# amoretti86/PSVO

Measured on AMD Instinct MI355X. Metric: particle-steps/sec, higher is better.
Workload: dtype f32

## Files before the change

psvo_amd/csrc/bsim_bwd2_impl.h:

```cpp
#pragma once
#define PSVO_BSIM_BWD_V2_UNIT 1
#include "bsim_bwd_impl.h"

namespace psvo {
PSVO_TIMERS_DEFINE(bsim_bwd2)

template <class T>
using gptr = T __attribute__((address_space(1)))*;
template <class T>
__device__ __forceinline__ gptr<T> as_global(T* p) { return (gptr<T>)p; }
template <class T>
__device__ __forceinline__ gptr<T> as_global(unsigned long long p) { return (gptr<T>)p; }
__device__ __forceinline__ float ldf(gptr<const float> base, unsigned off) {
    return *reinterpret_cast<gptr<const float>>(reinterpret_cast<gptr<const char>>(base) + off);
}
__device__ __forceinline__ int ldi(gptr<const int32_t> base, unsigned off) {
    return *reinterpret_cast<gptr<const int32_t>>(reinterpret_cast<gptr<const char>>(base) + off);
}
__device__ __forceinline__ void stf(gptr<float> base, unsigned off, float v) {
    *reinterpret_cast<gptr<float>>(reinterpret_cast<gptr<char>>(base) + off) = v;
}
#define PSVO_GARG(args_type, field) ::psvo::as_global(PSVO_ARG(args_type, field))

__device__ __forceinline__ float swap_add32(float lo, float hi) {
    asm volatile("s_nop 1\n\tv_permlane32_swap_b32 %0, %1" : "+v"(lo), "+v"(hi));
    return lo + hi;
}
__device__ __forceinline__ float swap_add16(float lo, float hi) {
    asm volatile("s_nop 1\n\tv_permlane16_swap_b32 %0, %1" : "+v"(lo), "+v"(hi));
    return lo + hi;
}
__device__ __forceinline__ float row_sum16(float v) {
    v += dpp_mov<0x128, 0xF, 0xF, true>(v, v);
    v += dpp_mov<0x124, 0xF, 0xF, true>(v, v);
    v += dpp_mov<0x122, 0xF, 0xF, true>(v, v);
    v += dpp_mov<0x121, 0xF, 0xF, true>(v, v);
    return v;
}

__device__ __forceinline__ float rs_bit3(float lo, float hi) {
    float r;
    asm volatile("s_nop 1\n\t"
                 "v_add_f32_dpp %0, %1, %1 row_ror:8 row_mask:0xf bank_mask:0x3\n\t"
                 "v_add_f32_dpp %0, %2, %2 row_ror:8 row_mask:0xf bank_mask:0xc"
                 : "=&v"(r) : "v"(lo), "v"(hi));
    return r;
}
__device__ __forceinline__ float rs_bit2(float lo, float hi) {
    float r;
    asm volatile("s_nop 1\n\t"
                 "v_add_f32_dpp %0, %1, %1 row_shl:4 row_mask:0xf bank_mask:0x5\n\t"
                 "v_add_f32_dpp %0, %2, %2 row_shr:4 row_mask:0xf bank_mask:0xa"
                 : "=&v"(r) : "v"(lo), "v"(hi));
    return r;
}
template <int K>
__device__ __forceinline__ void row_reduce_scatter(const float (&v)[4 * K], float (&out)[K]) {
    float h[2 * K];
#pragma unroll
    for (int i = 0; i < 2 * K; ++i) h[i] = rs_bit3(v[i], v[2 * K + i]);
#pragma unroll
    for (int i = 0; i < K; ++i) out[i] = group_sum<4>(rs_bit2(h[i], h[K + i]));
}

typedef float f4v __attribute__((ext_vector_type(4)));
typedef __bf16 bf8v __attribute__((ext_vector_type(8)));

__device__ __forceinline__ void bf16_split3(float v, unsigned& h, unsigned& m, unsigned& l) {
    const unsigned hb = __float_as_uint(v) & 0xffff0000u;
    const float r = v - __uint_as_float(hb);
    const unsigned mb = __float_as_uint(r) & 0xffff0000u;
    const float r2 = r - __uint_as_float(mb);
    h = hb >> 16;
    m = mb >> 16;
    l = __float_as_uint(r2) >> 16;
}
__device__ __forceinline__ uint4 bf16x3_a(float v) {
    unsigned h, m, l;
    bf16_split3(v, h, m, l);
    return make_uint4(h | (h << 16), m | (h << 16), l | (m << 16), m | (l << 16));
}
__device__ __forceinline__ uint4 bf16x3_b(float v) {
    unsigned h, m, l;
    bf16_split3(v, h, m, l);
    return make_uint4(h | (m << 16), h | (l << 16), h | (m << 16), l | (m << 16));
}

template <int DX, int DY, int H, int M, int JM>
__global__ void __launch_bounds__(256, 2) bsim_bwd2_kernel(const BsimBwdArgs a) {
    using MQ = MlpLds<DX, H, DX, 1>;
    using MG = MlpLds<DX, H, DY, 1>;
    using AC = BAcc<DX, DY>;
    constexpr int PS = (JM == 3) ? 20 : (DX == 4 && JM == 0) ? 5 : BTileSlot<DX>::kFloats;
    constexpr int FO = (JM == 3) ? 16 : 0;
    constexpr int NA = DX + 1;
    constexpr int PART = 2;
    constexpr int G = M * PART;
    constexpr int CPW = 64 / G;
    constexpr int CM = CPW * M;
    constexpr int NF = DX + 2;
    constexpr int UVS = (2 * DX + 3) & ~3;
    constexpr int JC = (JM == 0 && DX == 4) ? 2 : (JM || DX >= 3) ? 4 : 8;
    constexpr bool RO = (DX == 4) && (JM == 0);
    constexpr bool kSplitTile = (DX == 4) && (JM == 0);
    static_assert(CM == 32 && (M % 4) == 0, "two lanes per (chain, m): M in {4, 8, 16, 32}");
    extern __shared__ __attribute__((aligned(16))) float smem[];

    const int tid = threadIdx.x, lane = tid & 63, wave = tid >> 6;
    constexpr int NTB = 256, nwv = 4;
    const int B = a.B, T = a.T, N = a.N;
    const int NP = ((N + 127) / 128) * 128;
    const int nch = NP / (16 * JC);
    const int b = blockIdx.y, blk = blockIdx.x, nblk = gridDim.x;
    constexpr int cpb = nwv * CPW;
    const int cl = lane / G, part = (lane / M) & 1, m = lane % M;
    const bool h0 = (part == 0);
    const int n_raw = blk * cpb + wave * CPW + cl;
    const bool valid = n_raw < N;
    const int n = valid ? n_raw : N - 1;
    const bool srow = valid && h0;
    const bool lead = srow && (m == 0);
    const int j16 = lane & 15, g = lane >> 4;

    float* wf = smem;
    float* wg = wf + MQ::kSize;
    float* wqi = wg + MG::kSize;
    float* tile = wqi + MQ::kSize;
    float* jacc = tile + 2 * NP * PS;
    float* xch = jacc + nwv * NA * NP;
    float* uvx = xch + nwv * NF * CM;
    float* red = uvx + nwv * CM * UVS;
    float* const xw = xch + wave * NF * CM;
    float* const uw = uvx + wave * CM * UVS;
    float* const ja = jacc + wave * NA * NP;

    MQ::load(wf, a.f, tid, NTB);
    MG::load(wg, a.g, tid, NTB);
    MQ::load(wqi, a.q1inv, tid, NTB);

    const float kappa = sqrtf(0.5f * kLog2e);
    float isf[DX], rp[DX], isfk[DX], isg[DY];
#pragma unroll
    for (int d = 0; d < DX; ++d) {
        isf[d] = 1.f / a.sig_f[d];
        rp[d] = isf[d] * kappa;
        isfk[d] = isf[d] / kappa;
    }
    float ikap2 = 1.f / (kappa * kappa);
#pragma unroll
    for (int e = 0; e < DY; ++e) isg[e] = 1.f / a.sig_g[e];
    float pc[DX], pic[DX], pi1[DX], pi2[DX];
#pragma unroll
    for (int d = 0; d < DX; ++d) {
        pi1[d] = 1.f / a.sig_q1inv[d];
        pi2[d] = 1.f / a.sig_bq2[d];
        pic[d] = pi1[d] + pi2[d];
        pc[d] = 1.f / pic[d];
    }
    float s_init[DX], is_init[DX], i_isig[DX], im[DX], mi[DX];
#pragma unroll
    for (int d = 0; d < DX; ++d) {
        s_init[d] = a.sig_init[d];
        is_init[d] = 1.f / s_init[d];
        i_isig[d] = 1.f / a.isig[d];
        im[d] = a.imean[b * DX + d];
        mi[d] = a.minit[b * DX + d];
    }
    if constexpr (DX <= 2) {
        keep_in_vgpr(isf); keep_in_vgpr(rp); keep_in_vgpr(isfk); keep_in_vgpr(isg); keep_in_vgpr(ikap2);
        keep_in_vgpr(pc); keep_in_vgpr(pic); keep_in_vgpr(pi1); keep_in_vgpr(pi2);
    }
    const float ninf = -__builtin_huge_valf();
    const float aw = valid ? as_global(a.dscore)[(size_t)b * N + n] : 0.f;

// ... 769 lines not shown
```

psvo_amd/csrc/bsim_fwd.hip:

```cpp
#include "common.h"

namespace psvo {
inline namespace PSVO_LNS {
PSVO_TIMERS_DEFINE(bsim_fwd)


struct BsimArgs {
    int B, T, N;
    int emission;
    psvo_mlp f, g, q1inv;
    const float *X, *Fm, *logW, *lse;
    const float *sig_f, *sig_g, *sig_q1inv, *sig_bq2;
    const float *bmu2, *minit, *sig_init, *imean, *isig;
    const float *obs, *eps_b, *u_b;
    const int32_t* sel_in;
    float *bwX, *flp, *glp, *Omega;
    int32_t* sel_out;
    float* score;
    float *lam2_all, *om_all, *mu1_all;
};

template <int DX>
struct TileSlot {
    static constexpr int kFloats = (DX <= 3) ? 4 : 8;
};

__device__ __forceinline__ float quad_bcast(float v, int lane, int i) { return __shfl(v, (lane & ~3) | i); }

__device__ __forceinline__ void lse2_merge(float& m, float& s, float m2, float s2) {
    const float nm = fmaxf(m, m2);
    const float a = (m == nm) ? 1.f : exp2_fast(m - nm);
    const float b = (m2 == nm) ? 1.f : exp2_fast(m2 - nm);
    s = s * a + s2 * b;
    m = nm;
}

template <int DX, int DY, int H, int M, int HS>
__global__ void __launch_bounds__(256) bsim_fwd_kernel(const BsimArgs a) {
    using MQ = MlpLds<DX, H, DX, PSVO_L>;
    using MG = MlpLds<DX, H, DY, PSVO_L>;
    constexpr int PS = TileSlot<DX>::kFloats;
    constexpr int kMaxStage = 4;
    constexpr bool kRolled = (2 * MQ::kSize + MG::kSize) > 330;
    constexpr bool kPeel = (DX <= 3);
    extern __shared__ __attribute__((aligned(16))) float smem[];

    const int tid = threadIdx.x, lane = tid & 63;
    const int NTB = blockDim.x;
    const int B = a.B, T = a.T, N = a.N;
    const int NP = ((N + 16 * HS - 1) / (16 * HS)) * (16 * HS);
    const int b = blockIdx.y;
    constexpr int G = M * HS;
    const int cpb = NTB / G;
    const int cl = tid / G, hpart = (tid % G) / M, m = tid % M, q = m & 3;
    const bool lead = (m == 0) && (hpart == 0);
    const int n_raw = blockIdx.x * cpb + cl;
    const bool valid = n_raw < N;
    const int n = valid ? n_raw : N - 1;
    const int gbase = lane - m;

    float* wf = smem;
    float* wg = wf + MQ::kSize;
    float* wqi = wg + MG::kSize;
    float* tile = wqi + MQ::kSize;

    MQ::load(wf, a.f, tid, NTB);
    MG::load(wg, a.g, tid, NTB);
    MQ::load(wqi, a.q1inv, tid, NTB);

    float isf[DX], rp[DX], isg[DY];
    float kf = -DX * kHalfLog2Pi, kg = -DY * kHalfLog2Pi;
    const float rscale = sqrtf(0.5f * kLog2e);
#pragma unroll
    for (int d = 0; d < DX; ++d) {
        const float s = a.sig_f[d];
        isf[d] = 1.f / s;
        rp[d] = isf[d] * rscale;
        kf -= logf(s);
    }
#pragma unroll
    for (int e = 0; e < DY; ++e) {
        const float s = a.sig_g[e];
        isg[e] = 1.f / s;
        kg -= logf(s);
    }
    float pc[DX], pic[DX], pi1[DX], pi2[DX];
    float kq = -DX * kHalfLog2Pi;
#pragma unroll
    for (int d = 0; d < DX; ++d) {
        pi1[d] = 1.f / a.sig_q1inv[d];
        pi2[d] = 1.f / a.sig_bq2[d];
        pic[d] = pi1[d] + pi2[d];
        pc[d] = 1.f / pic[d];
        kq -= logf(pc[d]);
    }
    float s_init[DX], is_init[DX], i_isig[DX], im[DX], mi[DX];
    float kinit = -DX * kHalfLog2Pi, kiota = -DX * kHalfLog2Pi;
#pragma unroll
    for (int d = 0; d < DX; ++d) {
        s_init[d] = a.sig_init[d];
        is_init[d] = 1.f / s_init[d];
        kinit -= logf(s_init[d]);
        i_isig[d] = 1.f / a.isig[d];
        kiota -= logf(a.isig[d]);
        im[d] = a.imean[b * DX + d];
        mi[d] = a.minit[b * DX + d];
    }
    const float logM = logf((float)M);
    const float ninf = -__builtin_huge_valf();

    float st[kMaxStage][DX + 1], st_l = 0.f;
    auto stage_load = [&](int tt) {
        const size_t tb = (size_t)tt * B + b;
        st_l = a.lse[tb];
#pragma unroll
        for (int r = 0; r < kMaxStage; ++r) {
            const int j = tid + r * NTB;
            if (j < NP) {
                const int jc = j < N ? j : N - 1;
#pragma unroll
                for (int d = 0; d < DX; ++d) st[r][d] = a.Fm[(tb * DX + d) * N + jc];
                st[r][DX] = a.logW[tb * N + jc];
            }
        }
    };
    auto stage_store = [&](float* buf) {
#pragma unroll
        for (int r = 0; r < kMaxStage; ++r) {
            const int j = tid + r * NTB;
            if (j < NP) {
                float F[DX];
#pragma unroll
                for (int d = 0; d < DX; ++d) F[d] = st[r][d] * rp[d];
                const float W = j < N ? (st[r][DX] - st_l) * kLog2e : ninf;
                if constexpr (DX <= 3) {
                    float4 v;
                    v.x = F[0];
                    v.y = DX > 1 ? F[DX > 1 ? 1 : 0] : 0.f;
                    v.z = DX > 2 ? F[DX > 2 ? 2 : 0] : 0.f;
                    v.w = W;
                    *reinterpret_cast<float4*>(buf + j * PS) = v;
                } else {
                    *reinterpret_cast<float4*>(buf + j * PS) = make_float4(F[0], F[1], F[2], F[3]);
                    *reinterpret_cast<float4*>(buf + j * PS + 4) = make_float4(W, 0.f, 0.f, 0.f);
                }
            }
        }
    };

    if (T >= 2) {
        stage_load(T - 2);
        stage_store(tile);
    }

    float eps_c[DX], bmu_c[DX], obs_c[DY], u_c = 0.f;
    int sel_c = 0;
    auto load_inputs = [&](int t, float (&e)[DX], float (&bm)[DX], float (&o)[DY], float& uu, int& ss) {
        const size_t tb = (size_t)t * B + b;
#pragma unroll
        for (int d = 0; d < DX; ++d) {
            e[d] = a.eps_b[((tb * DX + d) * N + n) * M + m];
            bm[d] = a.bmu2[tb * DX + d];
        }
#pragma unroll
        for (int k = 0; k < DY; ++k) o[k] = a.obs[tb * DY + k];
        if (a.sel_in) ss = a.sel_in[tb * N + n];
        else uu = a.u_b[tb * N + n];
    };
    load_inputs(T - 1, eps_c, bmu_c, obs_c, u_c, sel_c);
    __syncthreads();

    float xp[DX];
#pragma unroll
    for (int d = 0; d < DX; ++d) xp[d] = 0.f;
    float score = 0.f;

    SEC_INIT(bsim_fwd)
    auto step = [&](auto last_tag, auto zero_tag, const int t) {
        SEC(0);
        const size_t tb = (size_t)t * B + b;
        const float* cur = tile + ((T - 1 - t) & 1) * NP * PS;
        float* nxt = tile + ((T - t) & 1) * NP * PS;
        const bool last = last_tag;
        const bool tzero = zero_tag;

        float eps_n[DX], bmu_n[DX], obs_n[DY], u_n = 0.f;
        int sel_n = 0;
        if (!tzero) load_inputs(t - 1, eps_n, bmu_n, obs_n, u_n, sel_n);
        if (t >= 2) stage_load(t - 2);

        SEC(1);
        float x[DX], q_lp;
        if (last) {
            float mu[DX];
#pragma unroll
            for (int d = 0; d < DX; ++d) {
                mu[d] = mi[d];
                x[d] = fmaf(s_init[d], eps_c[d], mu[d]);
            }
            q_lp = diag_lp<DX>(x, mu, is_init, kinit);
            if (a.mu1_all && valid && lead) {
#pragma unroll
                for (int d = 0; d < DX; ++d) a.mu1_all[(tb * DX + d) * N + n] = 0.f;
            }
        } else {
            float m1[DX], mu[DX];
            {
                constexpr int kQS = (H / 4 < G) ? H / 4 : G;
                MQ::template eval_part<kQS>(wqi, (tid % G) & (kQS - 1), xp, m1);
#pragma unroll
                for (int d = 0; d < DX; ++d) m1[d] = group_sum<kQS>(m1[d]);
            }
            if (a.mu1_all && valid && lead) {
#pragma unroll
                for (int d = 0; d < DX; ++d) a.mu1_all[(tb * DX + d) * N + n] = m1[d];
            }
#pragma unroll
            for (int d = 0; d < DX; ++d) {
                mu[d] = pc[d] * fmaf(pi1[d], m1[d], pi2[d] * bmu_c[d]);
                x[d] = fmaf(pc[d], eps_c[d], mu[d]);
            }
            q_lp = diag_lp<DX>(x, mu, pic, kq);
        }

        SEC(2);
        float phi = 0.f;
        if (!last) {
            float fmx[DX];
            if constexpr (HS == 1) {
                MQ::template eval<kRolled>(wf, x, fmx);
            } else {
                MQ::template eval_part<HS, ilog2(M)>(wf, hpart, x, fmx);
#pragma unroll
                for (int d = 0; d < DX; ++d) fmx[d] += xor_lane<M>(fmx[d]);
            }
            phi = diag_lp<DX>(xp, fmx, isf, kf);
        }
        float gm[DY];
        if constexpr (HS == 1) {
            MG::template eval<kRolled>(wg, x, gm);
        } else {
            MG::template eval_part<HS, ilog2(M)>(wg, hpart, x, gm);
#pragma unroll
            for (int k = 0; k < DY; ++k) gm[k] += xor_lane<M>(gm[k]);
        }
        if (a.emission) {
#pragma unroll
            for (int k = 0; k < DY; ++k) gm[k] = emis_mean(gm[k]);
        }
        const float g_lp = diag_lp<DY>(obs_c, gm, isg, kg);

        SEC(3);
        float lam;
        if (!tzero) {
            float xq[4][DX];
#pragma unroll
            for (int d = 0; d < DX; ++d) {
                float t4[4];
                quad_bcast4(x[d] * rp[d], t4);
#pragma unroll
                for (int i = 0; i < 4; ++i) xq[i][d] = t4[i];
            }
            f2 xa[DX], xb[DX];
#pragma unroll
            for (int d = 0; d < DX; ++d) {
                xa[d] = f2{xq[0][d], xq[1][d]};
                xb[d] = f2{xq[2][d], xq[3][d]};
            }
            f2 mxa = f2{ninf, ninf}, mxb = mxa, sma = f2{0.f, 0.f}, smb = sma;
            const int nqh = (NP >> 2) / HS;
            const int j0 = hpart * nqh;
            auto block = [&](auto jb_tag, int k0) {
                constexpr int JB = decltype(jb_tag)::value;
                f2 va[JB], vb[JB];
                f2 bma = f2{ninf, ninf}, bmb = bma;
#pragma unroll
                for (int c = 0; c < JB; ++c) {
                    const float* p = cur + ((j0 + k0 + c) * 4 + q) * PS;
                    float F[DX], W;
                    if constexpr (DX <= 3) {
                        const float4 sl = *reinterpret_cast<const float4*>(p);
                        F[0] = sl.x;
                        if (DX > 1) F[DX > 1 ? 1 : 0] = sl.y;
                        if (DX > 2) F[DX > 2 ? 2 : 0] = sl.z;
                        W = sl.w;
                    } else {
                        const float4 sl = *reinterpret_cast<const float4*>(p);
                        F[0] = sl.x; F[1] = sl.y; F[2] = sl.z; F[3] = sl.w;
                        W = p[4];
                    }
                    f2 la = f2{W, W}, lb = la;
#pragma unroll
                    for (int d = 0; d < DX; ++d) {
                        const f2 Fd = f2{F[d], F[d]};
                        const f2 ua = xa[d] - Fd, ub = xb[d] - Fd;
                        la = pk_fma(-ua, ua, la);
                        lb = pk_fma(-ub, ub, lb);
                    }
                    va[c] = la;
                    vb[c] = lb;
                    bma = pk_max(bma, la);
                    bmb = pk_max(bmb, lb);
                }
                const f2 nma = pk_max(mxa, bma), nmb = pk_max(mxb, bmb);
                const f2 ba = f2{nma.x == ninf ? 0.f : nma.x, nma.y == ninf ? 0.f : nma.y};
                const f2 bb = f2{nmb.x == ninf ? 0.f : nmb.x, nmb.y == ninf ? 0.f : nmb.y};
                const f2 ra = mxa - ba, rb = mxb - bb;
                sma = sma * f2{exp2_fast(ra.x), exp2_fast(ra.y)};
                smb = smb * f2{exp2_fast(rb.x), exp2_fast(rb.y)};
#pragma unroll
                for (int c = 0; c < JB; ++c) {
                    const f2 da = va[c] - ba, db = vb[c] - bb;
                    sma += f2{exp2_fast(da.x), exp2_fast(da.y)};
                    smb += f2{exp2_fast(db.x), exp2_fast(db.y)};
                }
                mxa = nma;
                mxb = nmb;
            };
            int k0 = 0;
            for (; k0 + 16 <= nqh; k0 += 16) block(std::integral_constant<int, 16>{}, k0);
            if (nqh - k0 >= 8) {
                block(std::integral_constant<int, 8>{}, k0);
                k0 += 8;
            }
            if (nqh - k0 >= 4) block(std::integral_constant<int, 4>{}, k0);
            SEC(4);
            const float mx[4] = {mxa.x, mxa.y, mxb.x, mxb.y};
            const float sm[4] = {sma.x, sma.y, smb.x, smb.y};
            float lm = ninf, ls = 0.f;
#pragma unroll
            for (int i = 0; i < 4; ++i) {
                float gm = fmaxf(mx[i], xor_lane<1>(mx[i]));
                gm = fmaxf(gm, xor_lane<2>(gm));
                if constexpr (HS == 2) gm = fmaxf(gm, xor_lane<M>(gm));
                const float base = (gm == ninf) ? 0.f : gm;
                float sc = sm[i] * exp2_fast(mx[i] - base);
                sc += xor_lane<1>(sc);
                sc += xor_lane<2>(sc);
                if constexpr (HS == 2) sc += xor_lane<M>(sc);
                if (i == q) {
                    lm = gm;
                    ls = sc;
                }
            }
            const float lam2 = lm + log2_fast(ls);
            lam = fmaf(kLn2, lam2, kf);
            if (a.lam2_all && valid && hpart == 0) a.lam2_all[(tb * N + n) * M + m] = lam2;
        } else {
            lam = diag_lp<DX>(x, im, i_isig, kiota);
        }

        SEC(5);
        const float om_raw = lam + phi + g_lp - q_lp;
        const float omx = group_max<M>(om_raw);
        const float pw = exp2_fast((om_raw - omx) * kLog2e);
        const float cdfv = group_incl_scan<M>(pw, m);
        const float total = __shfl(cdfv, gbase + M - 1);
        const float omega = om_raw - fmaf(kLn2, log2_fast(total), omx);
        if (a.om_all && valid && hpart == 0) a.om_all[(tb * N + n) * M + m] = omega;
        int sel;
        if (a.sel_in) {
            sel = sel_c;
        } else {
            const unsigned long long bal = __ballot(cdfv <= u_c * total);
            const unsigned long long mask = (M == 64) ? ~0ull : (((1ull << M) - 1ull) << gbase);
            sel = min((int)__popcll(bal & mask), M - 1);
        }
        const int src = gbase + sel;
        float xs[DX];
#pragma unroll
        for (int d = 0; d < DX; ++d) xs[d] = __shfl(x[d], src);
        const float om_s = __shfl(omega, src);
        const float phi_s = __shfl(phi, src);
        SEC(6);
        const float g_s = __shfl(g_lp, src);
        const float q_s = __shfl(q_lp, src);
        const float lam_s = __shfl(lam, src);
        const float Om = om_s + q_s + logM;

        if (valid && lead) {
#pragma unroll
            for (int d = 0; d < DX; ++d) a.bwX[(tb * DX + d) * N + n] = xs[d];
            a.glp[tb * N + n] = g_s;
            a.Omega[tb * N + n] = Om;
            a.sel_out[tb * N + n] = sel;
            if (!last) a.flp[(tb + B) * N + n] = phi_s;
            if (tzero) a.flp[(size_t)b * N + n] = lam_s;
        }
        score += g_s - Om + (last ? 0.f : phi_s) + (tzero ? lam_s : 0.f);

#pragma unroll
        for (int d = 0; d < DX; ++d) {
            xp[d] = xs[d];
            eps_c[d] = eps_n[d];
            bmu_c[d] = bmu_n[d];
        }
#pragma unroll
        for (int k = 0; k < DY; ++k) obs_c[k] = obs_n[k];
        u_c = u_n;
        sel_c = sel_n;

        SEC(7);
        if (t >= 2) stage_store(nxt);
        __syncthreads();
        SEC(8);
    };
    if constexpr (kPeel) {
        step(std::true_type{}, std::false_type{}, T - 1);
        for (int t = T - 2; t >= 1; --t) step(std::false_type{}, std::false_type{}, t);
        step(std::false_type{}, std::true_type{}, 0);
    } else {
        for (int t = T - 1; t >= 0; --t) step(t == T - 1, t == 0, t);
    }
    if (valid && lead) a.score[(size_t)b * N + n] = score;
}

template <int DX, int DY, int H, int M>
static int launch_bsim(const BsimArgs& a, hipStream_t stream) {
    using MQ = MlpLds<DX, H, DX, PSVO_L>;
    using MG = MlpLds<DX, H, DY, PSVO_L>;
    constexpr int PS = TileSlot<DX>::kFloats;
    const long long waves1 = ((long long)a.B * a.N * M + 63) / 64;
    const int HS = (waves1 < 2048 && 2 * M <= 64 && (H / 2) % 4 == 0 && (PSVO_L == 1 || g_tune_l2_split)) ? 2 : 1;
    const int NP = ((a.N + 16 * HS - 1) / (16 * HS)) * (16 * HS);
    int NTB = ((a.N * M * HS + 63) / 64) * 64;
    if (NTB > 256) NTB = 256;
    const int cpb = NTB / (M * HS);
    const size_t lds = sizeof(float) * (2 * MQ::kSize + MG::kSize + 2 * (size_t)NP * PS);
    dim3 grid((a.N + cpb - 1) / cpb, a.B);
    clear_hip_error();
    if (HS == 2) {
        if constexpr (2 * M <= 64 && (H / 2) % 4 == 0)
            hipLaunchKernelGGL((bsim_fwd_kernel<DX, DY, H, M, 2>), grid, dim3(NTB), lds, stream, a);
    } else {
        hipLaunchKernelGGL((bsim_fwd_kernel<DX, DY, H, M, 1>), grid, dim3(NTB), lds, stream, a);
    }
    return launch_status();
}

}
}

PSVO_L2_DECL(psvo_bsim_forward)
PSVO_ENTRY(psvo_bsim_forward)(const psvo_desc* desc, const float* X, const float* Fm, const float* logW,
                                 const float* lse, const psvo_mlp* f, const psvo_mlp* g, const psvo_mlp* q1_inv,
                                 const float* sig_f, const float* sig_g, const float* sig_q1inv,
                                 const float* sig_bq2, const float* bmu2, const float* minit,
                                 const float* sig_init, const float* imean, const float* isig, const float* obs,
                                 const float* eps_b, const float* u_b, const int32_t* sel_in, float* bwX,
                                 float* flp, float* glp, float* Omega, int32_t* sel_out, float* score,
                                 float* lam2_all, float* om_all, float* mu1_all,
                                 void* stream) {
    using namespace psvo;
    if (!desc_layers_ok(desc) || !desc_emission_ok(desc)) return PSVO_ERR_UNSUPPORTED;
#if PSVO_L == 1
    if (desc && desc->layers == 2)
        return psvo_bsim_forward_l2(desc, X, Fm, logW, lse, f, g, q1_inv, sig_f, sig_g, sig_q1inv, sig_bq2, bmu2,
            minit, sig_init, imean, isig, obs, eps_b, u_b, sel_in, bwX, flp, glp, Omega, sel_out, score, lam2_all,
            om_all, mu1_all, stream);
#endif
    if (!mlp_layers_ok(f) || !mlp_layers_ok(g) || !mlp_layers_ok(q1_inv)) return PSVO_ERR_INVALID;
    if (!desc || !Fm || !logW || !lse || !f || !g || !q1_inv || !sig_f || !sig_g || !sig_q1inv || !sig_bq2 ||
        !bmu2 || !minit || !sig_init || !imean || !isig || !obs || !eps_b || !bwX || !flp || !glp || !Omega ||
        !sel_out || !score)
        return PSVO_ERR_INVALID;
    if (!u_b && !sel_in) return PSVO_ERR_INVALID;
    if (desc->B <= 0 || desc->T < 2 || desc->N <= 0 || desc->M <= 0) return PSVO_ERR_INVALID;
    if (desc->N > 1024 || desc->B > 65535) return PSVO_ERR_UNSUPPORTED;
    (void)X;

    BsimArgs a;
    a.B = desc->B; a.T = desc->T; a.N = desc->N; a.emission = desc->emission;
    a.f = *f; a.g = *g; a.q1inv = *q1_inv;
    a.X = X; a.Fm = Fm; a.logW = logW; a.lse = lse;
    a.sig_f = sig_f; a.sig_g = sig_g; a.sig_q1inv = sig_q1inv; a.sig_bq2 = sig_bq2;
    a.bmu2 = bmu2; a.minit = minit; a.sig_init = sig_init; a.imean = imean; a.isig = isig;
    a.obs = obs; a.eps_b = eps_b; a.u_b = u_b; a.sel_in = sel_in;
    a.bwX = bwX; a.flp = flp; a.glp = glp; a.Omega = Omega; a.sel_out = sel_out; a.score = score;
    a.lam2_all = lam2_all; a.om_all = om_all; a.mu1_all = mu1_all;
    hipStream_t s = static_cast<hipStream_t>(stream);
    return dispatch_shape_m(desc->Dx, desc->Dy, desc->H, desc->M, [&](auto dx, auto dy, auto h, auto m) {
        return launch_bsim<dx(), dy(), h(), m()>(a, s); });
}
```

psvo_amd/csrc/common.h:

```cpp
#pragma once
#include <cstddef>
#include <type_traits>
#include <hip/hip_runtime.h>
#include <stdint.h>

#include "../../include/psvo_hip.h"

#ifndef PSVO_L
#define PSVO_L 1
#endif
#if PSVO_L == 1
#define PSVO_LNS l1
#define PSVO_ENTRY(name) extern "C" int name
#define PSVO_L2_DECL(name) extern "C" __attribute__((visibility("hidden"))) decltype(name) name##_l2;
#elif PSVO_L == 2
#define PSVO_LNS l2
#define PSVO_ENTRY(name) extern "C" __attribute__((visibility("hidden"))) int name##_l2
#define PSVO_L2_DECL(name)
#else
#error "PSVO_L must be 1 or 2"
#endif

namespace psvo {

constexpr float kLog2e = 1.4426950408889634f;
constexpr float kLn2 = 0.6931471805599453f;
constexpr float kHalfLog2Pi = 0.9189385332046727f;
constexpr int kWave = 64;

extern thread_local hipError_t g_last_hip_error;
inline void clear_hip_error() { (void)hipGetLastError(); }
inline int launch_status() {
    const hipError_t e = hipGetLastError();
    if (e != hipSuccess) g_last_hip_error = e;
    return e == hipSuccess ? PSVO_OK : PSVO_ERR_HIP;
}

inline bool desc_layers_ok(const psvo_desc* d) { return !d || (d->layers >= 0 && d->layers <= 2); }

inline bool desc_emission_ok(const psvo_desc* d, int max_emission = 1) {
    return !d || (d->emission >= 0 && d->emission <= max_emission);
}

extern int g_tune_l2_split;
extern int g_tune_filter_bwd_scan;

extern int g_tune_skew_pct;

__device__ __forceinline__ void phase_skew(int cycles) {
    unsigned hw;
    asm volatile("s_getreg_b32 %0, hwreg(HW_REG_HW_ID)" : "=s"(hw));
    if (cycles > 0 && ((hw >> 16) & 1u)) {
        for (int i = 0; i < cycles; i += 64 * 32) __builtin_amdgcn_s_sleep(32);
    }
}

inline bool mlp_layers_ok(const psvo_mlp* m) { return PSVO_L == 1 || !m || (m->Wh && m->bh); }

template <int V, int... Vs, class F>
static inline int pick(int v, F&& f) {
    if (v == V) return f(std::integral_constant<int, V>{});
    if constexpr (sizeof...(Vs) > 0) return pick<Vs...>(v, f);
    else return PSVO_ERR_UNSUPPORTED;
}
template <class F> static inline int pick_dx(int Dx, F&& f) { return pick<2, 3, 4>(Dx, f); }
template <class F> static inline int pick_dy(int Dy, F&& f) { return pick<1, 2>(Dy, f); }
template <class F> static inline int pick_m(int M, F&& f) { return pick<4, 8, 16, 32>(M, f); }
inline namespace PSVO_LNS {
template <class F> static inline int pick_h(int H, F&& f) {
#if PSVO_L == 1
    return pick<16, 32, 64>(H, f);
#else
    return pick<32, 64>(H, f);
#endif
}

template <class F> static inline int dispatch_dy_h(int Dy, int H, F&& f) {
    return pick_dy(Dy, [&](auto dy) { return pick_h(H, [&](auto h) { return f(dy, h); }); });
}
template <class F> static inline int dispatch_dy_h_m(int Dy, int H, int M, F&& f) {
    return dispatch_dy_h(Dy, H, [&](auto dy, auto h) { return pick_m(M, [&](auto m) { return f(dy, h, m); }); });
}
template <class F> static inline int dispatch_shape(int Dx, int Dy, int H, F&& f) {
    return pick_dx(Dx, [&](auto dx) { return dispatch_dy_h(Dy, H, [&](auto dy, auto h) { return f(dx, dy, h); }); });
}
template <class F> static inline int dispatch_shape_m(int Dx, int Dy, int H, int M, F&& f) {
    return pick_dx(Dx, [&](auto dx) { return dispatch_dy_h_m(Dy, H, M, [&](auto dy, auto h, auto m) { return f(dx, dy, h, m); }); });
}
}

static inline int wr_cluster(int B, int N, int M) {
    int K = 8;
    while (K > 1 && ((long long)B * K > 256 || N < 4 * K || (N + K - 1) / K * (K - 1) >= N)) K >>= 1;
    (void)M;
    return K;
}

#ifdef PSVO_SECTION_TIMERS
#define PSVO_TIMERS_DEFINE(name)                                                                        \
    __device__ unsigned long long g_sec_##name[32];                                                       \
    extern "C" int psvo_debug_timers_##name(unsigned long long* out, int reset) {                         \
        if (hipMemcpyFromSymbol(out, HIP_SYMBOL(g_sec_##name), 32 * sizeof(unsigned long long)) != hipSuccess) \
            return -1;                                                                                    \
        if (reset) {                                                                                      \
            unsigned long long z[32] = {0};                                                               \
            if (hipMemcpyToSymbol(HIP_SYMBOL(g_sec_##name), z, sizeof(z)) != hipSuccess) return -1;       \
        }                                                                                                 \
        return 0;                                                                                         \
    }
#define SEC_INIT(name)                                                                          \
    unsigned long long* const _sec = g_sec_##name;                                              \
    const bool _rec = (blockIdx.x == 0 && blockIdx.y == 0 && threadIdx.x == 0);                 \
    unsigned long long _tp = clock64();
#define SEC(i)                                   \
    do {                                         \
        const unsigned long long _tn = clock64(); \
        if (_rec) _sec[i] += _tn - _tp;          \
        _tp = _tn;                               \
    } while (0)
#else
#define PSVO_TIMERS_DEFINE(name)
#define SEC_INIT(name)
#define SEC(i)
#endif

__device__ __forceinline__ float exp2_fast(float x) { return __builtin_amdgcn_exp2f(x); }
__device__ __forceinline__ float log2_fast(float x) { return __builtin_amdgcn_logf(x); }

typedef float f2 __attribute__((ext_vector_type(2)));
__device__ __forceinline__ f2 pk_fma(f2 a, f2 b, f2 c) { return __builtin_elementwise_fma(a, b, c); }
__device__ __forceinline__ f2 pk_max(f2 a, f2 b) { return __builtin_elementwise_max(a, b); }
template <int HALF>
__device__ __forceinline__ f2 pk_fma_bcast(f2 a, f2 b, f2 c) {
    f2 d;
    if constexpr (HALF == 0)
        asm("v_pk_fma_f32 %0, %1, %2, %3 op_sel_hi:[0,1,1]" : "=v"(d) : "v"(a), "v"(b), "v"(c));
    else
        asm("v_pk_fma_f32 %0, %1, %2, %3 op_sel:[1,0,0] op_sel_hi:[1,1,1]" : "=v"(d) : "v"(a), "v"(b), "v"(c));
    return d;
}

__device__ __forceinline__ void keep_in_vgpr(float& x) { asm volatile("" : "+v"(x)); }
template <int K>
__device__ __forceinline__ void keep_in_vgpr(float (&x)[K]) {
#pragma unroll
    for (int i = 0; i < K; ++i) asm volatile("" : "+v"(x[i]));
}

template <class T>
__device__ __forceinline__ T* arg_ptr(unsigned byte_off) {
    asm volatile("" : "+s"(byte_off));
    typedef const char __attribute__((address_space(4))) * kptr;
    const kptr kp = (kptr)__builtin_amdgcn_kernarg_segment_ptr();
    typedef T* const __attribute__((address_space(4))) * pptr;
    return *(pptr)(kp + byte_off);
}
template <int NPTR>
__device__ __forceinline__ void arg_block(unsigned byte_off, unsigned long long (&out)[NPTR]) {
    static_assert(NPTR == 2 || NPTR == 4 || NPTR == 8, "pointer block of 2, 4 or 8");
    asm volatile("" : "+s"(byte_off));
    typedef const char __attribute__((address_space(4))) * kptr;
    const kptr kp = (kptr)__builtin_amdgcn_kernarg_segment_ptr();
    typedef unsigned long long vec_t __attribute__((ext_vector_type(NPTR)));
    typedef const vec_t __attribute__((address_space(4))) * vptr;
    const vec_t v = *(vptr)(kp + byte_off);
#pragma unroll
    for (int i = 0; i < NPTR; ++i) out[i] = v[i];
}
#define PSVO_ARG(args_type, field) \
    ::psvo::arg_ptr<std::remove_pointer_t<decltype(args_type::field)>>((unsigned)offsetof(args_type, field))

__device__ __forceinline__ float emis_mean(float r) { return (r > 20.f ? r : log1pf(expf(r))) + 1e-6f; }
__device__ __forceinline__ float emis_dmean(float r) { return 1.f / (1.f + expf(-r)); }

template <int DIN, int H, int DOUT, int L = 1>
struct MlpLds;

template <int DIN, int H, int DOUT>
struct MlpLds<DIN, H, DOUT, 1> {
    static constexpr int kW1 = 0;
    static constexpr int kB1 = DIN * H;
    static constexpr int kW2 = kB1 + H;
    static constexpr int kB2 = kW2 + DOUT * H;
    static constexpr int kSize = kB2 + ((DOUT + 3) & ~3);

    __device__ static void load(float* __restrict__ w, const psvo_mlp& p, int tid, int nthreads) {
        for (int i = tid; i < DIN * H; i += nthreads) w[kW1 + i] = p.W1[i];
        for (int i = tid; i < H; i += nthreads) w[kB1 + i] = p.b1[i];
        for (int i = tid; i < DOUT * H; i += nthreads) {
            const int o = i / H, k = i - o * H;
            w[kW2 + i] = p.W2[k * DOUT + o];
        }
        for (int i = tid; i < ((DOUT + 3) & ~3); i += nthreads) w[kB2 + i] = i < DOUT ? p.b2[i] : 0.f;
    }

    __device__ __forceinline__ static void group4(const float* __restrict__ w, int k, const float (&x)[DIN],
                                                  f2 (&acc)[DOUT]) {
        const float4 b = *reinterpret_cast<const float4*>(w + kB1 + k);
        f2 ha = f2{b.x, b.y}, hb = f2{b.z, b.w};
#pragma unroll
        for (int i = 0; i < DIN; ++i) {
            const float4 wi = *reinterpret_cast<const float4*>(w + kW1 + i * H + k);
            const f2 xi = f2{x[i], x[i]};
            ha = pk_fma(xi, f2{wi.x, wi.y}, ha);
            hb = pk_fma(xi, f2{wi.z, wi.w}, hb);
        }
        const f2 zero = f2{0.f, 0.f};
        ha = pk_max(ha, zero);
        hb = pk_max(hb, zero);
#pragma unroll
        for (int o = 0; o < DOUT; ++o) {
            const float4 wo = *reinterpret_cast<const float4*>(w + kW2 + o * H + k);
            acc[o] = pk_fma(ha, f2{wo.x, wo.y}, acc[o]);
            acc[o] = pk_fma(hb, f2{wo.z, wo.w}, acc[o]);
        }
    }

    template <bool ROLLED = false>
    __device__ __forceinline__ static void eval(const float* __restrict__ w, const float (&x)[DIN],
                                                float (&out)[DOUT]) {
        f2 acc[DOUT];
#pragma unroll
        for (int o = 0; o < DOUT; ++o) acc[o] = f2{w[kB2 + o], 0.f};
        if constexpr (ROLLED && (H % 8 == 0) && (H > 8)) {
#pragma unroll 1
            for (int k = 0; k < H; k += 8) {
                group4(w, k, x, acc);
                group4(w, k + 4, x, acc);
            }
        } else {
#pragma unroll
            for (int k = 0; k < H; k += 4) group4(w, k, x, acc);
        }
#pragma unroll
        for (int o = 0; o < DOUT; ++o) out[o] = acc[o].x + acc[o].y;
    }

    template <int S, int PB = 0>
    __device__ __forceinline__ static void eval_part(const float* __restrict__ w, int part, const float (&x)[DIN],
                                                     float (&out)[DOUT]) {
        constexpr int HP = H / S;
        static_assert(HP % 4 == 0, "hidden slice must be a multiple of 4");
        const float* wp = w + part * HP;
        f2 acc[DOUT];
#pragma unroll
        for (int o = 0; o < DOUT; ++o) acc[o] = f2{part == 0 ? w[kB2 + o] : 0.f, 0.f};
#pragma unroll
        for (int k = 0; k < HP; k += 4) group4(wp, k, x, acc);
#pragma unroll
        for (int o = 0; o < DOUT; ++o) out[o] = acc[o].x + acc[o].y;
    }

    __device__ __forceinline__ static void bwd_group4(const float* __restrict__ w, int k, const float (&x)[DIN],
                                                      const float (&dout)[DOUT], f2 (&dxa)[DIN]) {
        const float4 b = *reinterpret_cast<const float4*>(w + kB1 + k);
        f2 pa = f2{b.x, b.y}, pb = f2{b.z, b.w};
        f2 wa[DIN], wb[DIN];
#pragma unroll
        for (int i = 0; i < DIN; ++i) {
            const float4 wi = *reinterpret_cast<const float4*>(w + kW1 + i * H + k);
            wa[i] = f2{wi.x, wi.y};
            wb[i] = f2{wi.z, wi.w};
            const f2 xi = f2{x[i], x[i]};
            pa = pk_fma(xi, wa[i], pa);
            pb = pk_fma(xi, wb[i], pb);
        }
        f2 da = f2{0.f, 0.f}, db = da;
#pragma unroll
        for (int o = 0; o < DOUT; ++o) {
            const float4 wo = *reinterpret_cast<const float4*>(w + kW2 + o * H + k);
            const f2 go = f2{dout[o], dout[o]};
            da = pk_fma(go, f2{wo.x, wo.y}, da);
            db = pk_fma(go, f2{wo.z, wo.w}, db);
        }
        da = f2{pa.x > 0.f ? da.x : 0.f, pa.y > 0.f ? da.y : 0.f};
        db = f2{pb.x > 0.f ? db.x : 0.f, pb.y > 0.f ? db.y : 0.f};
#pragma unroll
        for (int i = 0; i < DIN; ++i) {
            dxa[i] = pk_fma(da, wa[i], dxa[i]);
            dxa[i] = pk_fma(db, wb[i], dxa[i]);
        }
    }

    template <int S, int PB = 0>
    __device__ __forceinline__ static void bwd_input_part(const float* __restrict__ w, int part, const float (&x)[DIN],
                                                          const float (&dout)[DOUT], float (&dx)[DIN]) {
        constexpr int HP = H / S;
        const float* wp = w + part * HP;
        f2 dxa[DIN];
#pragma unroll
        for (int i = 0; i < DIN; ++i) dxa[i] = f2{dx[i], 0.f};
#pragma unroll
        for (int k = 0; k < HP; k += 4) bwd_group4(wp, k, x, dout, dxa);
#pragma unroll
        for (int i = 0; i < DIN; ++i) dx[i] = dxa[i].x + dxa[i].y;
    }

    template <bool ROLLED = false>
    __device__ __forceinline__ static void bwd_input(const float* __restrict__ w, const float (&x)[DIN],
// ... 377 lines not shown
```

Before: 253.6 million.

## Rework bsim forward addressing with strength-reduced global pointers and register pinning

Replaces per-step 64-bit index arithmetic in the forward backward-simulation kernel with running global-address-space pointers that are decremented each time step, plus 32-bit byte offsets. Constants are pinned in VGPRs, store predicates are precomputed into a lane flag word, and prefetched inputs are 'settled' through an asm barrier so their loads complete at a chosen point. Launch bounds request two waves per SIMD for one L2 configuration. The aim is to cut scalar/vector address math and register pressure; it risks spills or altered scheduling, and moves the global pointer helpers into common.h.

Result: faster. 257.9 million, median of 6 (+1.7%).

```diff
diff --git a/psvo_amd/csrc/bsim_bwd2_impl.h b/psvo_amd/csrc/bsim_bwd2_impl.h
--- a/psvo_amd/csrc/bsim_bwd2_impl.h
+++ b/psvo_amd/csrc/bsim_bwd2_impl.h
@@ -5,21 +5,6 @@
 namespace psvo {
 PSVO_TIMERS_DEFINE(bsim_bwd2)
 
-template <class T>
-using gptr = T __attribute__((address_space(1)))*;
-template <class T>
-__device__ __forceinline__ gptr<T> as_global(T* p) { return (gptr<T>)p; }
-template <class T>
-__device__ __forceinline__ gptr<T> as_global(unsigned long long p) { return (gptr<T>)p; }
-__device__ __forceinline__ float ldf(gptr<const float> base, unsigned off) {
-    return *reinterpret_cast<gptr<const float>>(reinterpret_cast<gptr<const char>>(base) + off);
-}
-__device__ __forceinline__ int ldi(gptr<const int32_t> base, unsigned off) {
-    return *reinterpret_cast<gptr<const int32_t>>(reinterpret_cast<gptr<const char>>(base) + off);
-}
-__device__ __forceinline__ void stf(gptr<float> base, unsigned off, float v) {
-    *reinterpret_cast<gptr<float>>(reinterpret_cast<gptr<char>>(base) + off) = v;
-}
 #define PSVO_GARG(args_type, field) ::psvo::as_global(PSVO_ARG(args_type, field))
 
 __device__ __forceinline__ float swap_add32(float lo, float hi) {
diff --git a/psvo_amd/csrc/bsim_fwd.hip b/psvo_amd/csrc/bsim_fwd.hip
--- a/psvo_amd/csrc/bsim_fwd.hip
+++ b/psvo_amd/csrc/bsim_fwd.hip
@@ -36,7 +36,9 @@
 }
 
 template <int DX, int DY, int H, int M, int HS>
-__global__ void __launch_bounds__(256) bsim_fwd_kernel(const BsimArgs a) {
+constexpr int kBsimFwdWaves = (PSVO_L == 2 && DX == 2 && DY == 1 && H == 32 && !(M == 4 && HS == 1)) ? 2 : 1;
+template <int DX, int DY, int H, int M, int HS>
+__global__ void __launch_bounds__(256, (kBsimFwdWaves<DX, DY, H, M, HS>)) bsim_fwd_kernel(const BsimArgs a) {
     using MQ = MlpLds<DX, H, DX, PSVO_L>;
     using MG = MlpLds<DX, H, DY, PSVO_L>;
     constexpr int PS = TileSlot<DX>::kFloats;
@@ -106,29 +108,54 @@
         im[d] = a.imean[b * DX + d];
         mi[d] = a.minit[b * DX + d];
     }
-    const float logM = logf((float)M);
+    float logM = logf((float)M);
     const float ninf = -__builtin_huge_valf();
-
+    keep_in_vgpr(isf); keep_in_vgpr(rp); keep_in_vgpr(isg); keep_in_vgpr(pc); keep_in_vgpr(pic); keep_in_vgpr(pi1);
+    keep_in_vgpr(pi2); keep_in_vgpr(kf); keep_in_vgpr(kg); keep_in_vgpr(kq); keep_in_vgpr(logM);
+
+    typedef unsigned long long u64;
+    const u64 NM = (u64)N * M;
+    const unsigned s_1 = 4u * B, s_n = s_1 * N, s_d = s_1 * DX, s_k = s_1 * DY, s_dn = s_n * DX;
+    const u64 s_nm = s_1 * NM, s_dnm = s_nm * DX;
+    const u64 r_1 = 4ull * ((u64)(T - 1) * B + b);
+    const unsigned o_n = 4u * n, o_nm = 4u * (n * M + m), sN4 = 4u * N, sNM4 = 4u * N * M;
+    auto here = [](unsigned o) { asm volatile("" : "+v"(o)); return o; };
+    auto here_s = [](int v) { asm volatile("" : "+s"(v)); return v; };
+    const bool forced = a.sel_in != nullptr;
+    u64 p_eps = (u64)a.eps_b + r_1 * (DX * NM), p_bmu = (u64)a.bmu2 + r_1 * DX, p_obs = (u64)a.obs + r_1 * DY,
+        p_us = (forced ? (u64)a.sel_in : (u64)a.u_b) + r_1 * N;
+    u64 p_Fm = (u64)a.Fm + (r_1 - s_1) * (DX * N), p_logW = (u64)a.logW + (r_1 - s_1) * N, p_lse = (u64)a.lse + (r_1 - s_1);
+    constexpr unsigned kOut = 1u, kMu1 = 2u, kLam2 = 4u, kOm = 8u;
+    const unsigned lane_flags = (valid && lead ? kOut : 0u) | (a.mu1_all && valid && lead ? kMu1 : 0u) |
+                                (a.lam2_all && valid && hpart == 0 ? kLam2 : 0u) | (a.om_all && valid && hpart == 0 ? kOm : 0u);
+    auto stores = [&](unsigned bit) { return (here(lane_flags) & bit) != 0u; };
+    u64 p_bwX = (u64)a.bwX + r_1 * (DX * N), p_mu1 = (u64)a.mu1_all + r_1 * (DX * N), p_glp = (u64)a.glp + r_1 * N,
+        p_Om = (u64)a.Omega + r_1 * N, p_selo = (u64)a.sel_out + r_1 * N, p_flp = (u64)a.flp + r_1 * N,
+        p_lam2 = (u64)a.lam2_all + r_1 * NM, p_omall = (u64)a.om_all + r_1 * NM;
+
+    const int nsets = (NP + NTB - 1) / NTB;
     float st[kMaxStage][DX + 1], st_l = 0.f;
-    auto stage_load = [&](int tt) {
-        const size_t tb = (size_t)tt * B + b;
-        st_l = a.lse[tb];
+#pragma unroll
+    for (int r = 0; r < kMaxStage; ++r)
+#pragma unroll
+        for (int d = 0; d <= DX; ++d) st[r][d] = 0.f;
+    auto stage_load = [&]() {
+        st_l = ldf(as_global<const float>(p_lse), 0u);
 #pragma unroll
         for (int r = 0; r < kMaxStage; ++r) {
-            const int j = tid + r * NTB;
-            if (j < NP) {
-                const int jc = j < N ? j : N - 1;
-#pragma unroll
-                for (int d = 0; d < DX; ++d) st[r][d] = a.Fm[(tb * DX + d) * N + jc];
-                st[r][DX] = a.logW[tb * N + jc];
+            if (r == 0 || r < here_s(nsets)) {
+                const unsigned oj = here(4u * (unsigned)min(tid + r * NTB, N - 1));
+#pragma unroll
+                for (int d = 0; d < DX; ++d) st[r][d] = ldf(as_global<const float>(p_Fm), oj + d * sN4);
+                st[r][DX] = ldf(as_global<const float>(p_logW), oj);
             }
         }
     };
     auto stage_store = [&](float* buf) {
 #pragma unroll
         for (int r = 0; r < kMaxStage; ++r) {
-            const int j = tid + r * NTB;
-            if (j < NP) {
+            const int j = (int)here(tid) + r * NTB;
+            if ((r == 0 || r < here_s(nsets)) && j < NP) {
                 float F[DX];
 #pragma unroll
                 for (int d = 0; d < DX; ++d) F[d] = st[r][d] * rp[d];
@@ -148,26 +175,52 @@
         }
     };
 
-    if (T >= 2) {
-        stage_load(T - 2);
-        stage_store(tile);
-    }
-
-    float eps_c[DX], bmu_c[DX], obs_c[DY], u_c = 0.f;
-    int sel_c = 0;
-    auto load_inputs = [&](int t, float (&e)[DX], float (&bm)[DX], float (&o)[DY], float& uu, int& ss) {
-        const size_t tb = (size_t)t * B + b;
+    struct StepIn {
+        float eps[DX], bmu[DX], obs[DY];
+        int us;
+    };
+    auto load_inputs = [&](StepIn& s) {
 #pragma unroll
         for (int d = 0; d < DX; ++d) {
-            e[d] = a.eps_b[((tb * DX + d) * N + n) * M + m];
-            bm[d] = a.bmu2[tb * DX + d];
-        }
-#pragma unroll
-        for (int k = 0; k < DY; ++k) o[k] = a.obs[tb * DY + k];
-        if (a.sel_in) ss = a.sel_in[tb * N + n];
-        else uu = a.u_b[tb * N + n];
+            s.eps[d] = ldf(as_global<const float>(p_eps), here(o_nm) + d * sNM4);
+            s.bmu[d] = ldf(as_global<const float>(p_bmu), 4u * d);
+        }
+#pragma unroll
+        for (int k = 0; k < DY; ++k) s.obs[k] = ldf(as_global<const float>(p_obs), 4u * k);
+        s.us = ldi(as_global<const int32_t>(p_us), here(o_n));
     };
-    load_inputs(T - 1, eps_c, bmu_c, obs_c, u_c, sel_c);
+    auto settle = [&](StepIn& s) {
+        constexpr int kW = 2 * DX + DY + 2 + kMaxStage * (DX + 1);
+        float us = __int_as_float(s.us), pad = 0.f;
+        float* w[kW + 1];
+        int k = 0;
+#pragma unroll
+        for (int d = 0; d < DX; ++d) w[k++] = &s.eps[d];
+#pragma unroll
+        for (int d = 0; d < DX; ++d) w[k++] = &s.bmu[d];
+#pragma unroll
+        for (int e = 0; e < DY; ++e) w[k++] = &s.obs[e];
+        w[k++] = &us;
+        w[k++] = &st_l;
+#pragma unroll
+        for (int r = 0; r < kMaxStage; ++r)
+#pragma unroll
+            for (int d = 0; d <= DX; ++d) w[k++] = &st[r][d];
+        w[k++] = &pad;
+#pragma unroll
+        for (int i = 0; i + 1 < kW + 1; i += 2) {
+            f2 p = f2{*w[i], *w[i + 1]};
+            asm volatile("" : "+v"(p));
+            *w[i] = p.x;
+            *w[i + 1] = p.y;
+        }
+        s.us = __float_as_int(us);
+    };
+    StepIn cur_in;
+    load_inputs(cur_in);
+    stage_load();
+    settle(cur_in);
+    stage_store(tile);
     __syncthreads();
 
     float xp[DX];
@@ -178,16 +231,19 @@
     SEC_INIT(bsim_fwd)
     auto step = [&](auto last_tag, auto zero_tag, const int t) {
         SEC(0);
-        const size_t tb = (size_t)t * B + b;
         const float* cur = tile + ((T - 1 - t) & 1) * NP * PS;
         float* nxt = tile + ((T - t) & 1) * NP * PS;
         const bool last = last_tag;
         const bool tzero = zero_tag;
-
-        float eps_n[DX], bmu_n[DX], obs_n[DY], u_n = 0.f;
-        int sel_n = 0;
-        if (!tzero) load_inputs(t - 1, eps_n, bmu_n, obs_n, u_n, sel_n);
-        if (t >= 2) stage_load(t - 2);
+        constexpr bool kNoPrefetch = std::is_same<decltype(zero_tag), std::true_type>::value;
+        StepIn nxt_in;
+        if constexpr (!kNoPrefetch) {
+            const bool in_step = kPeel || t >= 1, tile_step = t >= 2;
+            p_eps -= in_step ? s_dnm : 0; p_bmu -= in_step ? s_d : 0; p_obs -= in_step ? s_k : 0; p_us -= in_step ? s_n : 0;
+            load_inputs(nxt_in);
+            p_Fm -= tile_step ? s_dn : 0; p_logW -= tile_step ? s_n : 0; p_lse -= tile_step ? s_1 : 0;
+            stage_load();
+        }
 
         SEC(1);
         float x[DX], q_lp;
@@ -196,12 +252,12 @@
 #pragma unroll
             for (int d = 0; d < DX; ++d) {
                 mu[d] = mi[d];
-                x[d] = fmaf(s_init[d], eps_c[d], mu[d]);
+                x[d] = fmaf(s_init[d], cur_in.eps[d], mu[d]);
             }
             q_lp = diag_lp<DX>(x, mu, is_init, kinit);
-            if (a.mu1_all && valid && lead) {
-#pragma unroll
-                for (int d = 0; d < DX; ++d) a.mu1_all[(tb * DX + d) * N + n] = 0.f;
+            if (stores(kMu1)) {
+#pragma unroll
+                for (int d = 0; d < DX; ++d) stf(as_global<float>(p_mu1), here(o_n) + d * sN4, 0.f);
             }
         } else {
             float m1[DX], mu[DX];
@@ -211,14 +267,14 @@
 #pragma unroll
                 for (int d = 0; d < DX; ++d) m1[d] = group_sum<kQS>(m1[d]);
             }
-            if (a.mu1_all && valid && lead) {
-#pragma unroll
-                for (int d = 0; d < DX; ++d) a.mu1_all[(tb * DX + d) * N + n] = m1[d];
+            if (stores(kMu1)) {
+#pragma unroll
+                for (int d = 0; d < DX; ++d) stf(as_global<float>(p_mu1), here(o_n) + d * sN4, m1[d]);
             }
 #pragma unroll
             for (int d = 0; d < DX; ++d) {
-                mu[d] = pc[d] * fmaf(pi1[d], m1[d], pi2[d] * bmu_c[d]);
-                x[d] = fmaf(pc[d], eps_c[d], mu[d]);
+                mu[d] = pc[d] * fmaf(pi1[d], m1[d], pi2[d] * cur_in.bmu[d]);
+                x[d] = fmaf(pc[d], cur_in.eps[d], mu[d]);
             }
             q_lp = diag_lp<DX>(x, mu, pic, kq);
         }
@@ -248,7 +304,7 @@
 #pragma unroll
             for (int k = 0; k < DY; ++k) gm[k] = emis_mean(gm[k]);
         }
-        const float g_lp = diag_lp<DY>(obs_c, gm, isg, kg);
+        const float g_lp = diag_lp<DY>(cur_in.obs, gm, isg, kg);
 
         SEC(3);
         float lam;
@@ -345,7 +401,7 @@
             }
             const float lam2 = lm + log2_fast(ls);
             lam = fmaf(kLn2, lam2, kf);
-            if (a.lam2_all && valid && hpart == 0) a.lam2_all[(tb * N + n) * M + m] = lam2;
+            if (stores(kLam2)) stf(as_global<float>(p_lam2), here(o_nm), lam2);
         } else {
             lam = diag_lp<DX>(x, im, i_isig, kiota);
         }
@@ -357,12 +413,12 @@
         const float cdfv = group_incl_scan<M>(pw, m);
         const float total = __shfl(cdfv, gbase + M - 1);
         const float omega = om_raw - fmaf(kLn2, log2_fast(total), omx);
-        if (a.om_all && valid && hpart == 0) a.om_all[(tb * N + n) * M + m] = omega;
+        if (stores(kOm)) stf(as_global<float>(p_omall), here(o_nm), omega);
         int sel;
-        if (a.sel_in) {
-            sel = sel_c;
+        if (forced) {
+            sel = cur_in.us;
         } else {
-            const unsigned long long bal = __ballot(cdfv <= u_c * total);
+            const unsigned long long bal = __ballot(cdfv <= __int_as_float(cur_in.us) * total);
             const unsigned long long mask = (M == 64) ? ~0ull : (((1ull << M) - 1ull) << gbase);
             sel = min((int)__popcll(bal & mask), M - 1);
         }
@@ -378,31 +434,28 @@
         const float lam_s = __shfl(lam, src);
         const float Om = om_s + q_s + logM;
 
-        if (valid && lead) {
-#pragma unroll
-            for (int d = 0; d < DX; ++d) a.bwX[(tb * DX + d) * N + n] = xs[d];
-            a.glp[tb * N + n] = g_s;
-            a.Omega[tb * N + n] = Om;
-            a.sel_out[tb * N + n] = sel;
-            if (!last) a.flp[(tb + B) * N + n] = phi_s;
-            if (tzero) a.flp[(size_t)b * N + n] = lam_s;
+        if constexpr (!kNoPrefetch) {
+            settle(nxt_in);
+            cur_in = nxt_in;
+        }
+        if (stores(kOut)) {
+            const unsigned on = here(o_n);
+#pragma unroll
+            for (int d = 0; d < DX; ++d) stf(as_global<float>(p_bwX), on + d * sN4, xs[d]);
+            stf(as_global<float>(p_glp), on, g_s);
+            stf(as_global<float>(p_Om), on, Om);
+            sti(as_global<int32_t>(p_selo), on, sel);
+            if (!last) stf(as_global<float>(p_flp + s_n), on, phi_s);
+            if (tzero) stf(as_global<float>(p_flp), on, lam_s);
         }
         score += g_s - Om + (last ? 0.f : phi_s) + (tzero ? lam_s : 0.f);
-
-#pragma unroll
-        for (int d = 0; d < DX; ++d) {
-            xp[d] = xs[d];
-            eps_c[d] = eps_n[d];
-            bmu_c[d] = bmu_n[d];
-        }
-#pragma unroll
-        for (int k = 0; k < DY; ++k) obs_c[k] = obs_n[k];
-        u_c = u_n;
-        sel_c = sel_n;
+#pragma unroll
+        for (int d = 0; d < DX; ++d) xp[d] = xs[d];
 
         SEC(7);
         if (t >= 2) stage_store(nxt);
         __syncthreads();
+        p_bwX -= s_dn; p_mu1 -= s_dn; p_glp -= s_n; p_Om -= s_n; p_selo -= s_n; p_flp -= s_n; p_lam2 -= s_nm; p_omall -= s_nm;
         SEC(8);
     };
     if constexpr (kPeel) {
diff --git a/psvo_amd/csrc/common.h b/psvo_amd/csrc/common.h
--- a/psvo_amd/csrc/common.h
+++ b/psvo_amd/csrc/common.h
@@ -145,6 +145,25 @@
 __device__ __forceinline__ void keep_in_vgpr(float (&x)[K]) {
 #pragma unroll
     for (int i = 0; i < K; ++i) asm volatile("" : "+v"(x[i]));
+}
+
+template <class T>
+using gptr = T __attribute__((address_space(1)))*;
+template <class T>
+__device__ __forceinline__ gptr<T> as_global(T* p) { return (gptr<T>)p; }
+template <class T>
+__device__ __forceinline__ gptr<T> as_global(unsigned long long p) { return (gptr<T>)p; }
+__device__ __forceinline__ float ldf(gptr<const float> base, unsigned off) {
+    return *reinterpret_cast<gptr<const float>>(reinterpret_cast<gptr<const char>>(base) + off);
+}
+__device__ __forceinline__ int ldi(gptr<const int32_t> base, unsigned off) {
+    return *reinterpret_cast<gptr<const int32_t>>(reinterpret_cast<gptr<const char>>(base) + off);
+}
+__device__ __forceinline__ void stf(gptr<float> base, unsigned off, float v) {
+    *reinterpret_cast<gptr<float>>(reinterpret_cast<gptr<char>>(base) + off) = v;
+}
+__device__ __forceinline__ void sti(gptr<int32_t> base, unsigned off, int v) {
+    *reinterpret_cast<gptr<int32_t>>(reinterpret_cast<gptr<char>>(base) + off) = v;
 }
 
 template <class T>
```
